# Fung-Lab/MatDeepLearn

Measured on AMD Instinct MI355X. Metric: edges/sec training CGCNN on bulk_data, higher is better.
Workload: dtype bf16

## Files before the change

include/mdl_hip.h:

```cpp
#ifndef MDL_HIP_H
#define MDL_HIP_H

#include <stddef.h>
#include <stdint.h>

#ifdef __cplusplus
extern "C" {
#endif

#define MDL_VERSION 100

enum { MDL_F32 = 0, MDL_BF16 = 1 };
enum { MDL_SUM = 0, MDL_MEAN = 1, MDL_MAX = 2 };
enum {
    MDL_OK = 0,
    MDL_E_ARG = -1,
    MDL_E_UNSUPP = -2,
    MDL_E_LAUNCH = -3
};

#define MDL_DTYPE_MASK 0xff
#define MDL_DETERMINISTIC 0x100
#define MDL_K3_PER_WAVE 0x200
#define MDL_K3_EDGE_LANE 0x400
#define MDL_BN_SHIFT_ROW 0x800
#define MDL_SPLIT_BF16 0x1000
#define MDL_MLP_F32_IO 0x2000

typedef void* mdlStream_t;

int mdl_version(void);
const char* mdl_last_error_string(void);
int mdl_debug_last_k3(void);

int mdl_rbf_expand(const float* d, const float* offsets, float coeff, void* out, int64_t E, int G,
                   int64_t ld_out, int out_dtype, mdlStream_t stream);

int mdl_csr_rowptr(const int32_t* sorted_index, int64_t E, int64_t N, int32_t* rowptr, mdlStream_t stream);

int mdl_segment_reduce_fwd(const void* src, const int32_t* rowptr, const int32_t* perm, void* out,
                           int32_t* argmax, int64_t N, int64_t C, int reduce, int dtype, mdlStream_t stream);
int mdl_segment_reduce_bwd(const void* grad_out, const int32_t* rowptr, const int32_t* seg,
                           const int32_t* perm, const int32_t* argmax, void* grad_src, int64_t N,
                           int64_t E, int64_t C, int reduce, int dtype, mdlStream_t stream);
int mdl_segment_reduce_bwd_add(const void* grad_out, const int32_t* rowptr, const int32_t* seg, const int32_t* perm,
                               const void* addend, void* grad_src, int64_t N, int64_t E, int64_t C, int reduce, int dtype,
                               mdlStream_t stream);

size_t mdl_cgconv_wpack_bytes(int C, int G, int dtype);
int mdl_cgconv_pack_weights(const float* w_f, const float* b_f, const float* w_s, const float* b_s, int C,
                            int G, void* wpack, float* bpack, int dtype, mdlStream_t stream);
int mdl_cgconv_pack_weights_node(const float* w_f, const float* b_f, const float* w_s, const float* b_s, int C,
                                 int G, void* wpack, float* bpack, void* wn_t, int dtype, mdlStream_t stream);

int mdl_cgconv_pack_weights_multi(int L, const float* const* w_f, const float* const* b_f, const float* const* w_s,
                                  const float* const* b_s, int C, int G, void* const* wpack, float* const* bpack,
                                  void* const* wn_t, int dtype, mdlStream_t stream);

int mdl_cgconv_fwd(const void* x, const void* edge_attr, const int32_t* rowptr, const int32_t* src,
                   const int32_t* tgt, const int32_t* eperm, const void* wpack, const float* bpack,
// ... 87 lines not shown
                       void* dh, void* dY, int64_t N, int Co, int D3, int dtype, mdlStream_t stream);

int mdl_pad_batch_tail(const int64_t* noff, const int64_t* eoff, int B, int64_t n_cap, int32_t* rowptr, int64_t* batch,
                       mdlStream_t stream);

int mdl_assemble_transposed(const int64_t* ids, const int64_t* noff, const int64_t* eoff, const int64_t* node_ptr,
                            const int64_t* edge_ptr, const int32_t* src_l, const int32_t* tgt_l, const int32_t* eperm_s,
                            const int32_t* lrowptr_s, int32_t* rowptr_s, int32_t* col_s, int32_t* eid_s, int32_t* src_s, int B,
                            int64_t n_cap, mdlStream_t stream);
int mdl_pad_edge_tail(const int64_t* noff, const int64_t* eoff, int B, int64_t n_cap, int64_t e_cap, int32_t* src, int32_t* tgt,
                      int32_t* col_s, int32_t* eid_s, int32_t* src_s, mdlStream_t stream);

int mdl_loss_fwd_bwd(const float* pred, const float* y, int64_t n, int kind, float* loss, float* grad, mdlStream_t stream);
int mdl_loss_fwd_bwd_rows(const float* pred, const float* y, int64_t n, int64_t n_total, int kind, float* loss, float* grad,
                          mdlStream_t stream);

#define MDL_BN_REPLICAS 16
int mdl_bn_sums_rows(void);
int mdl_bn_stats_n(const void* x, float* sums, int64_t N, int C, const int64_t* n_rows_dev, int dtype, mdlStream_t stream);
int mdl_bn_apply_n(const void* x, float* sums, const float* gamma, const float* beta, float* save, float* running_mean,
                   float* running_var, void* y, int64_t N, int C, float eps, float momentum, const int64_t* n_rows_dev,
                   int dtype, mdlStream_t stream);
int mdl_bn_bwd_stats_n(const void* dy, const void* x, const float* save, float* sums, int64_t N, int C,
                       const int64_t* n_rows_dev, int dtype, mdlStream_t stream);
int mdl_bn_bwd_apply_n(const void* dy, const void* x, const float* save, float* sums, const float* gamma, void* dx,
                       int64_t N, int C, const int64_t* n_rows_dev, int dtype, mdlStream_t stream);
int mdl_bn_bwd_apply_relu_n(const void* dy, const void* x, const float* save, float* sums, const float* gamma, void* dx,
                            int64_t N, int C, const int64_t* n_rows_dev, int dtype, mdlStream_t stream);
int mdl_linear_act(const void* x, const void* w, const void* bias, void* out, int64_t N, int K, int M, int act, int dtype,
                   mdlStream_t stream);
int mdl_linear_act_in(const void* x, const void* y, int xact, const void* w, const void* bias, void* out, int64_t N, int K,
                      int M, int act, int dtype, mdlStream_t stream);

int mdl_mlp_head_fwd(const void* x, const void* const* w, const void* const* b, void* const* h, int64_t N, int K0, int NL,
                     const int* M, int dtype, mdlStream_t stream);
int mdl_mlp_head_bwd(const void* x, const void* const* w, const void* const* h, const void* gy, void* dx, float* const* dw,
                     float* const* db, int64_t N, int K0, int NL, const int* M, int dtype, mdlStream_t stream);

int mdl_gru_gates_fwd(const void* gi, const void* gh, const float* h, float* h_out, void* out_lp, int64_t N, int C, int dtype,
                      mdlStream_t stream);
int mdl_gru_gates_bwd(const void* gi, const void* gh, const float* h, const float* g_h, const void* g_lp, void* dgi, void* dgh,
                      float* dh, int64_t N, int C, int dtype, mdlStream_t stream);

int mdl_linear_wide(const void* x, const void* w, void* out, int64_t N, int K, int64_t M, int dtype, mdlStream_t stream);

int mdl_gemm_tn(const void* a, int64_t lda, int M, const void* b, int64_t ldb, int K, float* c, int64_t N, int dtype,
                mdlStream_t stream);
int mdl_gemm_tn_colsum(const void* a, int64_t lda, int M, const void* b, int64_t ldb, int K, float* c, float* colsum,
                       int64_t N, int dtype, mdlStream_t stream);
int mdl_gemm_tn_act(const void* a, int64_t lda, int M, const void* y, int64_t ldy, int act, const void* b, int64_t ldb,
                    int K, float* c, float* colsum, int64_t N, int dtype, mdlStream_t stream);
int mdl_dense_bwd(const void* g, int64_t ldg, int M, const void* y, int64_t ldy, int act, const void* x, int64_t ldx, int K,
                  const void* w, void* dx, int64_t lddx, int xout, void* gm, float* dw, float* db, int64_t N, int dtype,
                  mdlStream_t stream);
size_t mdl_tn_scratch_bytes(void);
int mdl_dense_bwd_ex(const void* g, int64_t ldg, int M, const void* y, int64_t ldy, int act, const void* x, int64_t ldx, int K,
                     const void* w, void* dx, int64_t lddx, int xout, void* gm, float* dw, float* db, void* scratch, int64_t N,
                     int dtype, mdlStream_t stream);
int mdl_gemm_tn_ex(const void* a, int64_t lda, int M, const void* y, int64_t ldy, int act, const void* b, int64_t ldb, int K,
                   float* c, float* colsum, void* scratch, int64_t N, int dtype, mdlStream_t stream);

int mdl_gather_rows(const void* src, const int32_t* idx, void* out, int64_t E, int64_t C, int dtype,
                    mdlStream_t stream);
int mdl_gather_mul_reduce(const void* h, const void* w, const float* scale, const int32_t* rowptr,
                          const int32_t* col, const int32_t* eid, void* out, int64_t N, int64_t F, int reduce,
                          int dtype, mdlStream_t stream);
// ... 89 lines not shown
```

matdeeplearn_amd/_lib.py:

```python
import ctypes
import os

import torch

HERE = os.path.dirname(os.path.abspath(__file__))
LIB_PATH = os.path.join(HERE, "lib", "libmdl_hip.so")


def use_library(path):
    global LIB_PATH, _lib
    if _lib is not None and os.path.abspath(path) != os.path.abspath(LIB_PATH):
        raise MdlError("use_library(%s): %s is already loaded in this process" % (path, LIB_PATH))
    LIB_PATH = path

MDL_F32, MDL_BF16 = 0, 1
MDL_SUM, MDL_MEAN, MDL_MAX = 0, 1, 2
MDL_DTYPE_MASK, MDL_DETERMINISTIC, MDL_K3_PER_WAVE, MDL_K3_EDGE_LANE = 0xFF, 0x100, 0x200, 0x400
MDL_MLP_F32_IO = 0x2000
MDL_SPLIT_BF16 = 0x1000
MDL_BN_SHIFT_ROW = 0x800
MDL_BN_REPLICAS = 16
REDUCE = {"sum": MDL_SUM, "add": MDL_SUM, "mean": MDL_MEAN, "max": MDL_MAX}

_vp, _i64, _i32, _f32, _sz = ctypes.c_void_p, ctypes.c_int64, ctypes.c_int, ctypes.c_float, ctypes.c_size_t
_u32 = ctypes.c_uint32


class MdlCgConv(ctypes.Structure):
    _fields_ = [("size", _u32), ("dtype", _i32), ("flags", _u32), ("aggr", _i32), ("N", _i64), ("E", _i64), ("C", _i32), ("G", _i32),
                ("x", _vp), ("edge_attr", _vp), ("rowptr", _vp), ("src", _vp), ("tgt", _vp), ("eperm", _vp), ("wpack", _vp),
                ("bpack", _vp), ("out", _vp), ("bn_sums", _vp), ("bn_shift", _vp), ("bn_rows", _vp), ("grad_out", _vp),
                ("r_tgt", _vp), ("r_src", _vp), ("r_src_dtype", _i32), ("ld_dwe", _i32), ("dwe", _vp), ("db", _vp),
                ("workspace", _vp), ("workspace_bytes", _sz), ("balance", _vp)]


class MdlCgNode(ctypes.Structure):
    _fields_ = [("size", _u32), ("dtype", _i32), ("flags", _u32), ("zero_src", _i32), ("N", _i64), ("C", _i32), ("r_src_dtype", _i32),
                ("ld_dwn", _i32), ("reserved", _i32), ("x", _vp), ("grad_out", _vp), ("r_tgt", _vp), ("r_src", _vp), ("wn_t", _vp), ("dx", _vp), ("dwn", _vp)]


def _dp(t):
    return None if t is None else t.data_ptr()


def cg_args(**kw):
    a = MdlCgConv()
    a.size = ctypes.sizeof(MdlCgConv)
    for k, v in kw.items():
        setattr(a, k, _dp(v) if torch.is_tensor(v) else v)
    return a


def cg_node_args(**kw):
    a = MdlCgNode()
    a.size = ctypes.sizeof(MdlCgNode)
    for k, v in kw.items():
        setattr(a, k, _dp(v) if torch.is_tensor(v) else v)
    return a

PROTOTYPES = {
    "mdl_version": (_i32, []),
    "mdl_last_error_string": (ctypes.c_char_p, []),
    "mdl_debug_last_k3": (_i32, []),
    "mdl_rbf_expand": (_i32, [_vp, _vp, _f32, _vp, _i64, _i32, _i64, _i32, _vp]),
    "mdl_csr_rowptr": (_i32, [_vp, _i64, _i64, _vp, _vp]),
    "mdl_segment_reduce_fwd": (_i32, [_vp, _vp, _vp, _vp, _vp, _i64, _i64, _i32, _i32, _vp]),
    "mdl_segment_reduce_bwd": (_i32, [_vp, _vp, _vp, _vp, _vp, _vp, _i64, _i64, _i64, _i32, _i32, _vp]),
    "mdl_segment_reduce_bwd_add": (_i32, [_vp, _vp, _vp, _vp, _vp, _vp, _i64, _i64, _i64, _i32, _i32, _vp]),
    "mdl_cgconv_wpack_bytes": (_sz, [_i32, _i32, _i32]),
    "mdl_cgconv_pack_weights": (_i32, [_vp, _vp, _vp, _vp, _i32, _i32, _vp, _vp, _i32, _vp]),
    "mdl_cgconv_pack_weights_node": (_i32, [_vp, _vp, _vp, _vp, _i32, _i32, _vp, _vp, _vp, _i32, _vp]),
# ... 132 lines not shown
```

matdeeplearn_amd/csrc/mlp.hip:

```cpp
#include "mdl_common.h"

namespace mdl {

constexpr int MLP_MAXL = 4;
constexpr int MLP_LD = 72;

struct MlpArgs {
    const bf16_t* x;
    const bf16_t* w[MLP_MAXL];
    const bf16_t* b[MLP_MAXL];
    bf16_t* h[MLP_MAXL];
    const bf16_t* gy;
    bf16_t* dx;
    float* dw[MLP_MAXL];
    float* db[MLP_MAXL];
    int64_t N;
    int K0, NL;
    int M[MLP_MAXL];
    int f32io;
};

typedef __attribute__((ext_vector_type(4))) short s16x4;
typedef __attribute__((address_space(3))) s16x4* mlp_lds4_t;

__device__ __forceinline__ void mlp_stage(bf16_t* tile, const bf16_t* src, int64_t r0, int64_t N, int K, int tid) {
    if (K & 1) {
        bf16_t v[16];
#pragma unroll
        for (int u = 0; u < 16; ++u) {
            const int q = tid + 256 * u, row = q >> 6, c = q & 63;
            const bool ok = r0 + row < N && c < K;
            v[u] = src[ok ? (r0 + row) * (int64_t)K + c : 0];
        }
#pragma unroll
        for (int u = 0; u < 16; ++u) {
            const int q = tid + 256 * u, row = q >> 6, c = q & 63;
            tile[row * MLP_LD + c] = (r0 + row < N && c < K) ? v[u] : (bf16_t)0;
        }
        return;
    }
    const int k2 = K >> 1;
    unsigned v[8];
#pragma unroll
    for (int u = 0; u < 8; ++u) {
        const int q = tid + 256 * u, row = q >> 5, d = q & 31;
        const bool ok = r0 + row < N && d < k2;
        v[u] = *reinterpret_cast<const unsigned*>(src + (ok ? (r0 + row) * (int64_t)K + 2 * d : 0));
    }
#pragma unroll
    for (int u = 0; u < 8; ++u) {
        const int q = tid + 256 * u, row = q >> 5, d = q & 31;
        *reinterpret_cast<unsigned*>(tile + row * MLP_LD + 2 * d) = (r0 + row < N && d < k2) ? v[u] : 0u;
    }
}

__device__ __forceinline__ void mlp_stage_f32(bf16_t* tile, const float* src, int64_t r0, int64_t N, int K, int tid) {
    float v[16];
#pragma unroll
    for (int u = 0; u < 16; ++u) {
        const int q = tid + 256 * u, row = q >> 6, c = q & 63;
        const bool ok = r0 + row < N && c < K;
        v[u] = src[ok ? (r0 + row) * (int64_t)K + c : 0];
    }
#pragma unroll
    for (int u = 0; u < 16; ++u) {
        const int q = tid + 256 * u, row = q >> 6, c = q & 63;
        tile[row * MLP_LD + c] = (r0 + row < N && c < K) ? f2bf(v[u]) : (bf16_t)0;
    }
}

__device__ __forceinline__ f32x16 mlp_block(const bf16_t* tile_in, const bf16_t* wl, int mt, int nt, int i, int h, float bias) {
    f32x16 acc;
#pragma unroll
    for (int r = 0; r < 16; ++r) acc[r] = bias;
#pragma unroll
    for (int kk = 0; kk < 4; ++kk) {
        const bf16x8 a = *reinterpret_cast<const bf16x8*>(tile_in + (mt * 32 + i) * MLP_LD + 16 * kk + 8 * h);
        const bf16x8 b = *reinterpret_cast<const bf16x8*>(wl + (nt * 32 + i) * MLP_LD + 16 * kk + 8 * h);
        acc = __builtin_amdgcn_mfma_f32_32x32x16_bf16(a, b, acc, 0, 0, 0);
    }
    return acc;
}

__global__ __launch_bounds__(256, 2) void mlp_head_fwd_kernel(MlpArgs p) {
    extern __shared__ __attribute__((aligned(16))) char smem[];
    bf16_t* wl = reinterpret_cast<bf16_t*>(smem);
    bf16_t* ta = wl + p.NL * 64 * MLP_LD;
    bf16_t* tb = ta + 64 * MLP_LD;
    const int tid = threadIdx.x, lane = tid & 63, i = lane & 31, h = lane >> 5, wv = __builtin_amdgcn_readfirstlane(tid >> 6);
    const int mt = wv & 1, nt = wv >> 1;
    {
        unsigned wv_[MLP_MAXL][8];
#pragma unroll
        for (int l = 0; l < MLP_MAXL; ++l) {
            const int K = l < p.NL ? (l ? p.M[l - 1] : p.K0) : 0, M = l < p.NL ? p.M[l] : 0;
#pragma unroll
            for (int u = 0; u < 8; ++u) {
                const int q = tid + 256 * u, row = q >> 5, d = q & 31;
                unsigned v = 0u;
                if (row < M && 2 * d < K) v = *reinterpret_cast<const unsigned*>(p.w[l] + (int64_t)row * K + 2 * d);
                wv_[l][u] = v;
            }
        }
#pragma unroll
        for (int l = 0; l < MLP_MAXL; ++l) {
            if (l >= p.NL) break;
#pragma unroll
            for (int u = 0; u < 8; ++u) {
                const int q = tid + 256 * u, row = q >> 5, d = q & 31;
                *reinterpret_cast<unsigned*>(wl + (l * 64 + row) * MLP_LD + 2 * d) = wv_[l][u];
            }
        }
    }
    const int64_t n_tiles = (p.N + 63) / 64;
    for (int64_t tile = blockIdx.x; tile < n_tiles; tile += gridDim.x) {
        const int64_t r0 = tile * 64;
        __syncthreads();
        mlp_stage(ta, p.x, r0, p.N, p.K0, tid);
        __syncthreads();
        bf16_t* tin = ta;
        bf16_t* tout = tb;
        for (int l = 0; l < p.NL; ++l) {
            const int M = p.M[l], col = nt * 32 + i;
            const float bias = (p.b[l] && col < M) ? bf2f(p.b[l][col]) : 0.0f;
            const f32x16 acc = mlp_block(tin, wl + l * 64 * MLP_LD, mt, nt, i, h, bias);
            const bool relu = l + 1 < p.NL;
            bf16_t* const out = p.h[l];
            float* const out32 = (!relu && p.f32io) ? reinterpret_cast<float*>(p.h[l]) : nullptr;
#pragma unroll
            for (int r = 0; r < 16; ++r) {
                const int row = mt * 32 + 4 * h + (r & 3) + 8 * (r >> 2);
                float v = acc[r];
                if (relu) v = v > 0.0f ? v : 0.0f;
                const bf16_t hv = f2bf(v);
                tout[row * MLP_LD + col] = hv;
                if (col < M && r0 + row < p.N) {
                    if (out32) out32[(r0 + row) * (int64_t)M + col] = bf2f(hv);
                    else out[(r0 + row) * (int64_t)M + col] = hv;
                }
            }
            __syncthreads();
            bf16_t* t = tin; tin = tout; tout = t;
        }
    }
}

__global__ __launch_bounds__(256, 1) void mlp_head_bwd_kernel(MlpArgs p) {
    extern __shared__ __attribute__((aligned(16))) char smem[];
    bf16_t* wt = reinterpret_cast<bf16_t*>(smem);
    bf16_t* tin = wt + p.NL * 64 * MLP_LD;
    bf16_t* da = tin + p.NL * 64 * MLP_LD;
    bf16_t* dbuf = da + 64 * MLP_LD;
    const int tid = threadIdx.x, lane = tid & 63, i = lane & 31, h = lane >> 5, wv = __builtin_amdgcn_readfirstlane(tid >> 6);
    const int mt = wv & 1, nt = wv >> 1, t16 = i & 15;
    {
        unsigned wv_[MLP_MAXL][8];
#pragma unroll
        for (int l = 0; l < MLP_MAXL; ++l) {
            const int K = l < p.NL ? (l ? p.M[l - 1] : p.K0) : 0, M = l < p.NL ? p.M[l] : 0;
#pragma unroll
            for (int u = 0; u < 8; ++u) {
                const int q = tid + 256 * u, m = q >> 5, d = q & 31;
                unsigned v = 0u;
                if (m < M && 2 * d + 1 < K) v = *reinterpret_cast<const unsigned*>(p.w[l] + (int64_t)m * K + 2 * d);
                else if (m < M && 2 * d < K) v = (unsigned)p.w[l][(int64_t)m * K + 2 * d];
                wv_[l][u] = v;
            }
        }
#pragma unroll
        for (int l = 0; l < MLP_MAXL; ++l) {
            if (l >= p.NL) break;
#pragma unroll
            for (int u = 0; u < 8; ++u) {
                const int q = tid + 256 * u, m = q >> 5, d = q & 31;
                wt[(l * 64 + 2 * d) * MLP_LD + m] = (bf16_t)(wv_[l][u] & 0xffffu);
                wt[(l * 64 + 2 * d + 1) * MLP_LD + m] = (bf16_t)(wv_[l][u] >> 16);
            }
        }
    }
// ... 6 lines not shown
    const int64_t n_tiles = (p.N + 63) / 64;
    for (int64_t tile = blockIdx.x; tile < n_tiles; tile += gridDim.x) {
        const int64_t r0 = tile * 64;
        __syncthreads();
        for (int l = 0; l < p.NL; ++l)
            mlp_stage(tin + l * 64 * MLP_LD, l ? p.h[l - 1] : p.x, r0, p.N, l ? p.M[l - 1] : p.K0, tid);
        if (p.f32io) mlp_stage_f32(da, reinterpret_cast<const float*>(p.gy), r0, p.N, p.M[p.NL - 1], tid);
        else mlp_stage(da, p.gy, r0, p.N, p.M[p.NL - 1], tid);
        __syncthreads();
        bf16_t* dcur = da;
        bf16_t* dnext = dbuf;
#pragma unroll
        for (int lq = 0; lq < MLP_MAXL; ++lq) {
            const int l = p.NL - 1 - lq;
            if (l < 0) break;
            const bf16_t* const in = tin + l * 64 * MLP_LD;
#pragma unroll
            for (int ks = 0; ks < 4; ++ks) {
                const int roff = 16 * ks + 8 * h + (t16 >> 2), coff = (i & 16) + 4 * (t16 & 3);
                const bf16_t* pa = dcur + roff * MLP_LD + mt * 32 + coff;
                const bf16_t* pb = in + roff * MLP_LD + nt * 32 + coff;
                const s16x4 a0 = __builtin_amdgcn_ds_read_tr16_b64_v4i16((mlp_lds4_t)pa), a1 = __builtin_amdgcn_ds_read_tr16_b64_v4i16((mlp_lds4_t)(pa + 4 * MLP_LD));
                const s16x4 b0 = __builtin_amdgcn_ds_read_tr16_b64_v4i16((mlp_lds4_t)pb), b1 = __builtin_amdgcn_ds_read_tr16_b64_v4i16((mlp_lds4_t)(pb + 4 * MLP_LD));
                const bf16x8 af = {a0[0], a0[1], a0[2], a0[3], a1[0], a1[1], a1[2], a1[3]};
                const bf16x8 bf = {b0[0], b0[1], b0[2], b0[3], b1[0], b1[1], b1[2], b1[3]};
                dwacc[lq] = __builtin_amdgcn_mfma_f32_32x32x16_bf16(af, bf, dwacc[lq], 0, 0, 0);
            }
            {
                float s = 0.0f;
#pragma unroll
                for (int r = 0; r < 16; ++r) s += bf2f(dcur[(16 * (tid >> 6) + r) * MLP_LD + (tid & 63)]);
                dbacc[lq] += s;
            }
            if (l > 0 || p.dx) {
                const f32x16 acc = mlp_block(dcur, wt + l * 64 * MLP_LD, mt, nt, i, h, 0.0f);
                const int col = nt * 32 + i, K = l ? p.M[l - 1] : p.K0;
#pragma unroll
                for (int r = 0; r < 16; ++r) {
                    const int row = mt * 32 + 4 * h + (r & 3) + 8 * (r >> 2);
                    if (l > 0) {
                        const bool on = bf2f(in[row * MLP_LD + col]) > 0.0f;
                        dnext[row * MLP_LD + col] = f2bf(on ? acc[r] : 0.0f);
                    } else if (col < K && r0 + row < p.N) {
                        p.dx[(r0 + row) * (int64_t)K + col] = f2bf(acc[r]);
                    }
                }
            }
            __syncthreads();
            bf16_t* t = dcur; dcur = dnext; dnext = t;
        }
    }
    {
        float* red = reinterpret_cast<float*>(da);
        __syncthreads();
#pragma unroll
        for (int lq = 0; lq < MLP_MAXL; ++lq) red[(lq * 4 + (tid >> 6)) * 64 + (tid & 63)] = dbacc[lq];
        __syncthreads();
#pragma unroll
        for (int lq = 0; lq < MLP_MAXL; ++lq)
            dbacc[lq] = tid < 64 ? ((red[(lq * 4 + 0) * 64 + tid] + red[(lq * 4 + 1) * 64 + tid]) + red[(lq * 4 + 2) * 64 + tid]) + red[(lq * 4 + 3) * 64 + tid] : 0.0f;
    }
#pragma unroll
    for (int lq = 0; lq < MLP_MAXL; ++lq) {
        const int l = p.NL - 1 - lq;
        if (l < 0) break;
        const int K = l ? p.M[l - 1] : p.K0, M = p.M[l], k = nt * 32 + i;
#pragma unroll
        for (int r = 0; r < 16; ++r) {
            const int m = mt * 32 + 4 * h + (r & 3) + 8 * (r >> 2);
            if (m < M && k < K) unsafeAtomicAdd(p.dw[l] + (int64_t)m * K + k, dwacc[lq][r]);
        }
        if (tid < 64 && tid < M && p.db[l]) unsafeAtomicAdd(p.db[l] + tid, dbacc[lq]);
    }
}

static int mlp_check(const char* name, const MlpArgs& a, int dtype) {
    MDL_REQUIRE(dtype == MDL_BF16, MDL_E_UNSUPP, "%s: bf16 only", name);
    MDL_REQUIRE(a.NL >= 1 && a.NL <= MLP_MAXL && a.K0 >= 2 && a.K0 <= 64 && a.K0 % 2 == 0, MDL_E_UNSUPP,
                "%s: 1..4 dense layers, even input width <= 64 (got %d layers, K0 = %d)", name, a.NL, a.K0);
    for (int l = 0; l < a.NL; ++l) {
        MDL_REQUIRE(a.M[l] >= 1 && a.M[l] <= 64 && (l + 1 == a.NL || a.M[l] % 2 == 0), MDL_E_UNSUPP,
                    "%s: widths <= 64, hidden widths even (layer %d: %d)", name, l, a.M[l]);
        MDL_REQUIRE(a.w[l] && reinterpret_cast<uintptr_t>(a.w[l]) % 4 == 0, MDL_E_ARG, "%s: null / misaligned weight %d", name, l);
    }
    MDL_REQUIRE(a.N >= 0 && (a.N == 0 || (a.x && reinterpret_cast<uintptr_t>(a.x) % 4 == 0)), MDL_E_ARG, "%s: bad arguments", name);
    return MDL_OK;
}

}

extern "C" int mdl_mlp_head_fwd(const void* x, const void* const* w, const void* const* b, void* const* h, int64_t N, int K0,
                                int NL, const int* M, int dtype, mdlStream_t stream) {
    using namespace mdl;
    MlpArgs a = {};
    a.x = (const bf16_t*)x; a.N = N; a.K0 = K0; a.NL = NL;
    MDL_REQUIRE(NL >= 1 && NL <= MLP_MAXL && w && b && h && M, MDL_E_ARG, "mdl_mlp_head_fwd: bad arguments");
    for (int l = 0; l < NL; ++l) { a.w[l] = (const bf16_t*)w[l]; a.b[l] = (const bf16_t*)b[l]; a.h[l] = (bf16_t*)h[l]; a.M[l] = M[l]; }
    a.f32io = (dtype & MDL_MLP_F32_IO) != 0;
    dtype &= MDL_DTYPE_MASK;
    int rc = mlp_check("mdl_mlp_head_fwd", a, dtype);
    if (rc) return rc;
    for (int l = 0; l < NL; ++l) MDL_REQUIRE(N == 0 || a.h[l], MDL_E_ARG, "mdl_mlp_head_fwd: null output %d", l);
    if (N == 0) return MDL_OK;
    const int lds = (NL + 2) * 64 * MLP_LD * 2;
    hipError_t e = set_max_dynamic_lds(reinterpret_cast<const void*>(mlp_head_fwd_kernel), lds);
    if (e != hipSuccess) { set_error("mdl_mlp_head_fwd: LDS attribute (%d B): %s", lds, hipGetErrorString(e)); return MDL_E_LAUNCH; }
    int64_t grid = cdiv(N, 64);
    if (grid > 512) grid = 512;
    hipLaunchKernelGGL(mlp_head_fwd_kernel, dim3((unsigned)grid), dim3(256), lds, (hipStream_t)stream, a);
    return check_launch("mdl_mlp_head_fwd");
}

extern "C" int mdl_mlp_head_bwd(const void* x, const void* const* w, const void* const* h, const void* gy, void* dx,
                                float* const* dw, float* const* db, int64_t N, int K0, int NL, const int* M, int dtype,
                                mdlStream_t stream) {
    using namespace mdl;
    MlpArgs a = {};
    a.x = (const bf16_t*)x; a.gy = (const bf16_t*)gy; a.dx = (bf16_t*)dx; a.N = N; a.K0 = K0; a.NL = NL;
    MDL_REQUIRE(NL >= 1 && NL <= MLP_MAXL && w && h && dw && db && M, MDL_E_ARG, "mdl_mlp_head_bwd: bad arguments");
    for (int l = 0; l < NL; ++l) {
        a.w[l] = (const bf16_t*)w[l]; a.M[l] = M[l]; a.dw[l] = dw[l]; a.db[l] = db[l];
        a.h[l] = l + 1 < NL ? (bf16_t*)const_cast<void*>(h[l]) : nullptr;
    }
    const bool det = (dtype & MDL_DETERMINISTIC) != 0;
    a.f32io = (dtype & MDL_MLP_F32_IO) != 0;
    dtype &= MDL_DTYPE_MASK;
    int rc = mlp_check("mdl_mlp_head_bwd", a, dtype);
    if (rc) return rc;
    MDL_REQUIRE(N == 0 || (gy && reinterpret_cast<uintptr_t>(gy) % ((M[NL - 1] % 2 && !a.f32io) ? 2 : 4) == 0), MDL_E_ARG,
                "mdl_mlp_head_bwd: null / misaligned gy");
    for (int l = 0; l < NL; ++l) {
        MDL_REQUIRE(N == 0 || a.dw[l], MDL_E_ARG, "mdl_mlp_head_bwd: null dw %d", l);
        MDL_REQUIRE(N == 0 || l + 1 == NL || (a.h[l] && reinterpret_cast<uintptr_t>(a.h[l]) % 4 == 0), MDL_E_ARG, "mdl_mlp_head_bwd: null h %d", l);
    }
    if (N == 0) return MDL_OK;
    const int lds = (2 * NL + 2) * 64 * MLP_LD * 2;
    hipError_t e = set_max_dynamic_lds(reinterpret_cast<const void*>(mlp_head_bwd_kernel), lds);
    if (e != hipSuccess) { set_error("mdl_mlp_head_bwd: LDS attribute (%d B): %s", lds, hipGetErrorString(e)); return MDL_E_LAUNCH; }
    int64_t grid = cdiv(N, 64);
    if (grid > 256) grid = 256;
    if (det) grid = 1;
    hipLaunchKernelGGL(mlp_head_bwd_kernel, dim3((unsigned)grid), dim3(256), lds, (hipStream_t)stream, a);
    return check_launch("mdl_mlp_head_bwd");
}
```

matdeeplearn_amd/models/_base.py:

```python
import torch
import torch.nn.functional as F
from torch import nn

from .. import ops
from ..nn import BatchNorm1d, Set2Set, lowp_copies as _lowp


def dense(lin, h, split=False):
    if h.dtype == lin.weight.dtype:
        if split and ops.linear_split_ok(h, lin.weight):
            return ops._LinearSplitTN.apply(h, lin.weight, lin.bias)
        return lin(h)
    return ops.linear(h, lin.weight, lin.bias, _lowp(lin))


def dense_act(lin, h, act, split=False):
    if h.dtype == lin.weight.dtype:
        return getattr(F, act)(dense(lin, h, split))
    return ops.linear_act(h, lin.weight, lin.bias, act, _lowp(lin))


class GraphModel(nn.Module):

    def _begin(self, data, dim1, pre_fc_count, gc_count, pool, pool_order, batch_norm, batch_track_stats, act,
# ... 75 lines not shown
        ops.new_grad_arena(device, n)

    def _pre(self, out):
        if torch.is_grad_enabled() and out.is_cuda:
            self._open_grad_arena(out.device)
        if out.dtype == torch.bfloat16 and torch.is_grad_enabled():
            self._cast_dense(out.dtype)
        for lin in self.pre_lin_list:
            out = dense_act(lin, out, self.act, split=self.split_products)
        return out

    def _bn(self, i, out):
        return self.bn_list[i](out) if self.batch_norm == "True" else out

    def _drop(self, out):
        return F.dropout(out, p=self.dropout_rate, training=self.training)

    def _post(self, out, final=False):
        lins = list(self.post_lin_list) + [self.lin_out]
        if out.dtype != self.lin_out.weight.dtype and ops.mlp_head_ok(out, lins, self.act):
            return ops.mlp_head(out, lins, [_lowp(lin) for lin in lins], f32_out=final)
        for lin in self.post_lin_list:
            out = dense_act(lin, out, self.act, split=self.split_products)
        return dense(self.lin_out, out)

    def _pool(self, out, data):
        num_graphs = getattr(data, "num_graphs", None)
        if self.pool == "set2set":
            return self.set2set(out, data.batch, num_graphs)
        return ops.POOLS[self.pool](out, data.batch, num_graphs, seg_index=getattr(data, "pool_index", None))

    def _head(self, out, data):
        if self.pool_order == "early":
            out = self._post(self._pool(out, data).to(out.dtype), final=True)
        else:
            out = self._post(out)
            if self.pool == "set2set":
                out = dense(self.lin_out_2, self._pool(out, data).to(out.dtype))
            else:
                out = self._pool(out, data)
        out = out.float()
        return out.view(-1) if out.shape[1] == 1 else out
```

matdeeplearn_amd/ops.py:

```python
import collections
import os
import weakref

import torch

from . import _lib
from ._lib import MdlError, check, dtype_code, lib, ptr, require_hip, stream

_ACT_CODE = {"relu": 1, "ssp": 2}
_LN2 = 0.6931471805599453


def _f32c(t):
    return None if t is None else t.detach().float().contiguous()


def _stream_key(device):
    return (device.index, torch.cuda.current_stream(device).cuda_stream)


class EdgeCSR:

    __slots__ = ("rowptr", "src", "tgt", "eperm", "N", "E", "_row", "_col", "_t", "_attr", "_tb", "_bal", "partial", "__weakref__")

# ... 484 lines not shown
    prev, _DET = _DET, bool(on)
    return prev


class deterministic:
    def __init__(self, on=True):
        self.on = on

    def __enter__(self):
        self.prev = set_deterministic(self.on)
        return self

    def __exit__(self, *exc):
        set_deterministic(self.prev)
        return False


OPTIONS = {
    "deterministic": ("_DET", "bit-reproducible launch shapes of every atomically accumulating kernel (slow; HIP-vs-HIP tests)"),
    "gmr_dw": ("_GMR_DW", "CFConv backward: dh and dw from one walk over the by-source CSR"),
    "balance": ("_BALANCE", "cost-balanced node ranges for the edge-per-lane CGConv backward (E >= 4e5)"),
    "pad128": ("_PAD128", "C in (96, 128): static 128-channel CGConv kernels on zero-padded rows"),
    "rsrc16": ("_RSRC16", "by-source sums of the CGConv backward in bf16 (packed atomics)"),
    "cg_bn_stats": ("_CG_BN_STATS", "BatchNorm statistics in the CGConv forward's epilogue (measured time-neutral: off)"),
    "direct_grads": ("_DIRECT_GRADS", "K3 / K3c add into the final dW layout (measured slower at small batches: off)"),
    "cfconv_fused": ("_CFCONV_FUSED", "K4: the fused CFConv forward"),
    "cfconv_recompute": ("_CFCONV_RECOMPUTE", "K4b: CFConv backward with the filter recomputed (no per-edge activations)"),
    "tn_colsum": ("_TN_COLSUM", "bias gradients out of the TN GEMM"),
    "dense_bwd": ("_DENSE_BWD", "dX + dW + db of a tall dense layer in one pass"),
    "dense_bwd_wide": ("_DENSE_BWD_WIDE", "... also when both widths exceed 128"),
    "mlp_head": ("_MLP_HEAD", "post-FC head as one launch per direction"),
    "linear_wide": ("_LINEAR_WIDE", "NNConv's Y = x W2r on the streaming kernel"),
    "set2set_fused": ("_SET2SET_FUSED", "Set2Set readout: all processing steps in one launch per direction (off: torch's LSTM + the composed attention)"),
    "tn_scratch": ("_TN_SCRATCH", "weight-gradient blocks of the TN products as plain stores + a reduce launch (off: atomics from every workgroup)"),
}


def configure(**kw):
    prev = {}
    g = globals()
    for k, v in kw.items():
        if k not in OPTIONS:
            raise MdlError("ops.configure: unknown option %r (known: %s)" % (k, ", ".join(sorted(OPTIONS))))
        attr = OPTIONS[k][0]
        prev[k] = g[attr]
        g[attr] = bool(v)
    return prev


def options():
    return {k: globals()[a] for k, (a, _) in OPTIONS.items()}


def _dflag():
    return _lib.MDL_DETERMINISTIC if _DET else 0


K3_VARIANT = None


def _k3flag():
    return {None: 0, "per_wave": _lib.MDL_K3_PER_WAVE, "edge_lane": _lib.MDL_K3_EDGE_LANE}[K3_VARIANT]


def last_k3():
    return int(lib().mdl_debug_last_k3())
# ... 1008 lines not shown
            flat, dbv = _dw_db_zeros(M[l], Ks[l], x.device)
            dws.append(flat.view(M[l], Ks[l]))
            dbs.append(dbv if ctx.has_bias[l] else None)
        dx = torch.empty_like(x) if ctx.needs_input_grad[0] else None
        Ma = (ctypes.c_int * NL)(*M)
        check(lib().mdl_mlp_head_bwd(ptr(x), _ptr_array(ws), _ptr_array(hs + [None]), ptr(gy), ptr(dx), _ptr_array(dws), _ptr_array(dbs),
                                     N, K0, NL, Ma, dtype_code(x) | _dflag() | ctx.io, stream()), "mdl_mlp_head_bwd")
        grads = []
        for l in range(NL):
            grads.append(dws[l].to(ctx.wdtypes[l]))
            grads.append(dbs[l].to(ctx.wdtypes[l]) if ctx.has_bias[l] else None)
        return (dx, None, None) + tuple(grads)


def mlp_head_ok(x, lins, act):
    if not (_MLP_HEAD and act == "relu" and x.dtype == torch.bfloat16 and x.is_cuda and x.dim() == 2 and x.is_contiguous()
            and 1 <= len(lins) <= 4 and x.shape[0] >= 1 and x.shape[1] <= 64 and x.shape[1] % 2 == 0 and x.data_ptr() % 4 == 0):
        return False
    k = x.shape[1]
    for j, lin in enumerate(lins):
        if lin.in_features != k or lin.out_features > 64 or (j + 1 < len(lins) and lin.out_features % 2) or not lin.weight.requires_grad:
            return False
        k = lin.out_features
    return True


def mlp_head(x, lins, lowp=None, f32_out=False):
    params = []
    for lin in lins:
        params += [lin.weight, lin.bias]
    return _MlpHead.apply(x, lowp, bool(f32_out), *params)


class _LinearWide(torch.autograd.Function):

    @staticmethod
    def forward(ctx, x, w):
        N, K = x.shape
        M = w.shape[1]
        wt = w.t().contiguous()
        out = torch.empty((N, M), dtype=x.dtype, device=x.device)
        check(lib().mdl_linear_wide(ptr(x), ptr(wt), ptr(out), N, K, M, dtype_code(x), stream()), "mdl_linear_wide")
        ctx.save_for_backward(x, w)
        return out

    @staticmethod
    def backward(ctx, g):
        x, w = ctx.saved_tensors
        dx = g @ w.t() if ctx.needs_input_grad[0] else None
        dw = x.t() @ g if ctx.needs_input_grad[1] else None
        return dx, dw


def matmul_wide(x, w):
    if (_LINEAR_WIDE and x.dtype == torch.bfloat16 and w.dtype == torch.bfloat16 and x.is_cuda and x.dim() == 2 and x.is_contiguous()
            and x.shape[0] >= 1024 and x.shape[1] % 2 == 0 and 4 <= x.shape[1] <= 160 and w.shape[1] >= 640
            and x.data_ptr() % 16 == 0):
        return _LinearWide.apply(x, w)
    return x @ w


def linear_act_fused_ok(x, weight, act):
    return (x.dtype == torch.bfloat16 and x.is_cuda and x.dim() == 2 and x.is_contiguous() and x.shape[0] >= _DENSE_MIN_ROWS
            and _fused_fwd_shape_ok(weight.shape[0], weight.shape[1], act) and x.data_ptr() % 16 == 0 and weight.requires_grad)


# ... 872 lines not shown
```

Measured before the change: 819.8 million.

## Fuse graph pooling into the MLP head kernels for forward and backward

Adds an MDL_MLP_POOL mode in which the MLP head forward kernel sums or averages each graph's node rows straight into its LDS tile, using 512 threads where the extra waves help with the gather. The backward kernel scatters the first-layer input gradient back to the node rows. This removes the separate segment-reduce launch and its backward, along with the pooled-tensor round trips. The cost is a larger forward block with half the waves idle during the GEMM stage, and an imbalanced per-graph node loop.

Result: no change. 822.7 million, median of 6 (+0.4%).

```diff
diff --git a/include/mdl_hip.h b/include/mdl_hip.h
--- a/include/mdl_hip.h
+++ b/include/mdl_hip.h
@@ -26,6 +26,7 @@
 #define MDL_BN_SHIFT_ROW 0x800
 #define MDL_SPLIT_BF16 0x1000
 #define MDL_MLP_F32_IO 0x2000
+#define MDL_MLP_POOL 0x4000
 
 typedef void* mdlStream_t;
 
@@ -179,6 +180,14 @@
 int mdl_linear_act_in(const void* x, const void* y, int xact, const void* w, const void* bias, void* out, int64_t N, int K,
                       int M, int act, int dtype, mdlStream_t stream);
 
+typedef struct MdlReadout {
+    uint32_t size;
+    int32_t pool;
+    int64_t n_nodes;
+    const int32_t* node_ptr;
+    const void* x;
+    void* pooled;
+} MdlReadout;
 int mdl_mlp_head_fwd(const void* x, const void* const* w, const void* const* b, void* const* h, int64_t N, int K0, int NL,
                      const int* M, int dtype, mdlStream_t stream);
 int mdl_mlp_head_bwd(const void* x, const void* const* w, const void* const* h, const void* gy, void* dx, float* const* dw,
diff --git a/matdeeplearn_amd/_lib.py b/matdeeplearn_amd/_lib.py
--- a/matdeeplearn_amd/_lib.py
+++ b/matdeeplearn_amd/_lib.py
@@ -17,6 +17,7 @@
 MDL_SUM, MDL_MEAN, MDL_MAX = 0, 1, 2
 MDL_DTYPE_MASK, MDL_DETERMINISTIC, MDL_K3_PER_WAVE, MDL_K3_EDGE_LANE = 0xFF, 0x100, 0x200, 0x400
 MDL_MLP_F32_IO = 0x2000
+MDL_MLP_POOL = 0x4000
 MDL_SPLIT_BF16 = 0x1000
 MDL_BN_SHIFT_ROW = 0x800
 MDL_BN_REPLICAS = 16
@@ -37,6 +38,17 @@
 class MdlCgNode(ctypes.Structure):
     _fields_ = [("size", _u32), ("dtype", _i32), ("flags", _u32), ("zero_src", _i32), ("N", _i64), ("C", _i32), ("r_src_dtype", _i32),
                 ("ld_dwn", _i32), ("reserved", _i32), ("x", _vp), ("grad_out", _vp), ("r_tgt", _vp), ("r_src", _vp), ("wn_t", _vp), ("dx", _vp), ("dwn", _vp)]
+
+
+class MdlReadout(ctypes.Structure):
+    _fields_ = [("size", _u32), ("pool", _i32), ("n_nodes", _i64), ("node_ptr", _vp), ("x", _vp), ("pooled", _vp)]
+
+
+def readout_args(pool, n_nodes, node_ptr, x, pooled):
+    a = MdlReadout()
+    a.size, a.pool, a.n_nodes = ctypes.sizeof(MdlReadout), pool, n_nodes
+    a.node_ptr, a.x, a.pooled = _dp(node_ptr), _dp(x), _dp(pooled)
+    return a
 
 
 def _dp(t):
diff --git a/matdeeplearn_amd/csrc/mlp.hip b/matdeeplearn_amd/csrc/mlp.hip
--- a/matdeeplearn_amd/csrc/mlp.hip
+++ b/matdeeplearn_amd/csrc/mlp.hip
@@ -18,7 +18,15 @@
     int K0, NL;
     int M[MLP_MAXL];
     int f32io;
+    const int32_t* node_ptr;
+    const bf16_t* xn;
+    bf16_t* pooled;
+    bf16_t* dxn;
+    int64_t NN;
+    int mean;
 };
+
+typedef __attribute__((ext_vector_type(4))) unsigned mlp_u32x4;
 
 typedef __attribute__((ext_vector_type(4))) short s16x4;
 typedef __attribute__((address_space(3))) s16x4* mlp_lds4_t;
@@ -54,6 +62,76 @@
     }
 }
 
+template <int NT>
+__device__ __forceinline__ void mlp_stage_pool(bf16_t* tile, const MlpArgs& p, int64_t r0, int tid) {
+    constexpr int S = 512 / NT, U = 16 / S;
+    int b[S], n[S];
+    float acc[S][8];
+#pragma unroll
+    for (int s = 0; s < S; ++s) {
+        const int g = (tid + NT * s) >> 3;
+        const bool ok = r0 + g < p.N;
+        const int64_t lo = ok ? p.node_ptr[r0 + g] : 0, hi = ok ? p.node_ptr[r0 + g + 1] : 0;
+        b[s] = (int)(lo < 0 ? 0 : (lo > p.NN ? p.NN : lo));
+        n[s] = (int)((hi > p.NN ? p.NN : hi) - b[s]);
+        if (n[s] < 0) n[s] = 0;
+#pragma unroll
+        for (int j = 0; j < 8; ++j) acc[s][j] = 0.0f;
+    }
+    const bf16_t* const base = p.xn + (tid & 7) * 8;
+    const int nmax = n[0] > n[S - 1] ? n[0] : n[S - 1];
+    for (int k = 0; k < nmax; k += U) {
+        bf16x8 v[S][U];
+#pragma unroll
+        for (int s = 0; s < S; ++s)
+#pragma unroll
+            for (int u = 0; u < U; ++u) {
+                int kk = b[s] + (k + u < n[s] ? k + u : n[s] - 1);
+                if (kk < 0) kk = 0;
+                v[s][u] = *reinterpret_cast<const bf16x8*>(base + (int64_t)kk * 64);
+            }
+#pragma unroll
+        for (int s = 0; s < S; ++s)
+#pragma unroll
+            for (int u = 0; u < U; ++u)
+                if (k + u < n[s]) {
+#pragma unroll
+                    for (int j = 0; j < 8; ++j) acc[s][j] += bf2f((bf16_t)v[s][u][j]);
+                }
+    }
+#pragma unroll
+    for (int s = 0; s < S; ++s) {
+        const int q = tid + NT * s, g = q >> 3, c8 = q & 7;
+        if (p.mean) {
+            const float cnt = (float)(n[s] > 1 ? n[s] : 1);
+#pragma unroll
+            for (int j = 0; j < 8; ++j) acc[s][j] = acc[s][j] / cnt;
+        }
+        const mlp_u32x4 r = {pk_bf16(acc[s][0], acc[s][1]), pk_bf16(acc[s][2], acc[s][3]), pk_bf16(acc[s][4], acc[s][5]), pk_bf16(acc[s][6], acc[s][7])};
+        *reinterpret_cast<mlp_u32x4*>(tile + g * MLP_LD + c8 * 8) = r;
+        if (r0 + g < p.N) *reinterpret_cast<mlp_u32x4*>(p.pooled + (r0 + g) * 64 + c8 * 8) = r;
+    }
+}
+
+__device__ __forceinline__ void mlp_unpool(const bf16_t* tile, const MlpArgs& p, int64_t r0, int tid) {
+#pragma unroll
+    for (int s = 0; s < 2; ++s) {
+        const int q = tid + 256 * s, g = q >> 3, c8 = q & 7;
+        if (r0 + g >= p.N) continue;
+        const int64_t lo = p.node_ptr[r0 + g], hi = p.node_ptr[r0 + g + 1];
+        const int64_t b = lo < 0 ? 0 : (lo > p.NN ? p.NN : lo), e = hi > p.NN ? p.NN : hi;
+        float v[8];
+        Vec<bf16_t>::ld(tile + g * MLP_LD + c8 * 8, v);
+        if (p.mean) {
+            const float cnt = (float)(e - b > 1 ? e - b : 1);
+#pragma unroll
+            for (int j = 0; j < 8; ++j) v[j] = v[j] / cnt;
+        }
+        const mlp_u32x4 r = {pk_bf16(v[0], v[1]), pk_bf16(v[2], v[3]), pk_bf16(v[4], v[5]), pk_bf16(v[6], v[7])};
+        for (int64_t k = b; k < e; ++k) *reinterpret_cast<mlp_u32x4*>(p.dxn + k * 64 + c8 * 8) = r;
+    }
+}
+
 __device__ __forceinline__ void mlp_stage_f32(bf16_t* tile, const float* src, int64_t r0, int64_t N, int K, int tid) {
     float v[16];
 #pragma unroll
@@ -82,14 +160,15 @@
     return acc;
 }
 
-__global__ __launch_bounds__(256, 2) void mlp_head_fwd_kernel(MlpArgs p) {
+template <bool POOL>
+__global__ __launch_bounds__(POOL ? 512 : 256, POOL ? 1 : 2) void mlp_head_fwd_kernel(MlpArgs p) {
     extern __shared__ __attribute__((aligned(16))) char smem[];
     bf16_t* wl = reinterpret_cast<bf16_t*>(smem);
     bf16_t* ta = wl + p.NL * 64 * MLP_LD;
     bf16_t* tb = ta + 64 * MLP_LD;
     const int tid = threadIdx.x, lane = tid & 63, i = lane & 31, h = lane >> 5, wv = __builtin_amdgcn_readfirstlane(tid >> 6);
     const int mt = wv & 1, nt = wv >> 1;
-    {
+    if (!POOL || tid < 256) {
         unsigned wv_[MLP_MAXL][8];
 #pragma unroll
         for (int l = 0; l < MLP_MAXL; ++l) {
@@ -116,27 +195,30 @@
     for (int64_t tile = blockIdx.x; tile < n_tiles; tile += gridDim.x) {
         const int64_t r0 = tile * 64;
         __syncthreads();
-        mlp_stage(ta, p.x, r0, p.N, p.K0, tid);
+        if constexpr (POOL) mlp_stage_pool<512>(ta, p, r0, tid);
+        else mlp_stage(ta, p.x, r0, p.N, p.K0, tid);
         __syncthreads();
         bf16_t* tin = ta;
         bf16_t* tout = tb;
         for (int l = 0; l < p.NL; ++l) {
             const int M = p.M[l], col = nt * 32 + i;
-            const float bias = (p.b[l] && col < M) ? bf2f(p.b[l][col]) : 0.0f;
-            const f32x16 acc = mlp_block(tin, wl + l * 64 * MLP_LD, mt, nt, i, h, bias);
             const bool relu = l + 1 < p.NL;
             bf16_t* const out = p.h[l];
             float* const out32 = (!relu && p.f32io) ? reinterpret_cast<float*>(p.h[l]) : nullptr;
-#pragma unroll
-            for (int r = 0; r < 16; ++r) {
-                const int row = mt * 32 + 4 * h + (r & 3) + 8 * (r >> 2);
-                float v = acc[r];
-                if (relu) v = v > 0.0f ? v : 0.0f;
-                const bf16_t hv = f2bf(v);
-                tout[row * MLP_LD + col] = hv;
-                if (col < M && r0 + row < p.N) {
-                    if (out32) out32[(r0 + row) * (int64_t)M + col] = bf2f(hv);
-                    else out[(r0 + row) * (int64_t)M + col] = hv;
+            if (!POOL || wv < 4) {
+                const float bias = (p.b[l] && col < M) ? bf2f(p.b[l][col]) : 0.0f;
+                const f32x16 acc = mlp_block(tin, wl + l * 64 * MLP_LD, mt, nt, i, h, bias);
+#pragma unroll
+                for (int r = 0; r < 16; ++r) {
+                    const int row = mt * 32 + 4 * h + (r & 3) + 8 * (r >> 2);
+                    float v = acc[r];
+                    if (relu) v = v > 0.0f ? v : 0.0f;
+                    const bf16_t hv = f2bf(v);
+                    tout[row * MLP_LD + col] = hv;
+                    if (col < M && r0 + row < p.N) {
+                        if (out32) out32[(r0 + row) * (int64_t)M + col] = bf2f(hv);
+                        else out[(r0 + row) * (int64_t)M + col] = hv;
+                    }
                 }
             }
             __syncthreads();
@@ -145,6 +227,7 @@
     }
 }
 
+template <bool POOL>
 __global__ __launch_bounds__(256, 1) void mlp_head_bwd_kernel(MlpArgs p) {
     extern __shared__ __attribute__((aligned(16))) char smem[];
     bf16_t* wt = reinterpret_cast<bf16_t*>(smem);
@@ -217,7 +300,7 @@
                 for (int r = 0; r < 16; ++r) s += bf2f(dcur[(16 * (tid >> 6) + r) * MLP_LD + (tid & 63)]);
                 dbacc[lq] += s;
             }
-            if (l > 0 || p.dx) {
+            if (l > 0 || p.dx || POOL) {
                 const f32x16 acc = mlp_block(dcur, wt + l * 64 * MLP_LD, mt, nt, i, h, 0.0f);
                 const int col = nt * 32 + i, K = l ? p.M[l - 1] : p.K0;
 #pragma unroll
@@ -226,6 +309,8 @@
                     if (l > 0) {
                         const bool on = bf2f(in[row * MLP_LD + col]) > 0.0f;
                         dnext[row * MLP_LD + col] = f2bf(on ? acc[r] : 0.0f);
+                    } else if constexpr (POOL) {
+                        dnext[row * MLP_LD + col] = f2bf(acc[r]);
                     } else if (col < K && r0 + row < p.N) {
                         p.dx[(r0 + row) * (int64_t)K + col] = f2bf(acc[r]);
                     }
@@ -234,6 +319,7 @@
             __syncthreads();
             bf16_t* t = dcur; dcur = dnext; dnext = t;
         }
+        if constexpr (POOL) mlp_unpool(dcur, p, r0, tid);
     }
     {
         float* red = reinterpret_cast<float*>(da);
@@ -274,57 +360,100 @@
 
 }
 
-extern "C" int mdl_mlp_head_fwd(const void* x, const void* const* w, const void* const* b, void* const* h, int64_t N, int K0,
-                                int NL, const int* M, int dtype, mdlStream_t stream) {
+static int mlp_fwd_launch(const char* name, mdl::MlpArgs& a, const void* const* w, const void* const* b, void* const* h, int NL,
+                          const int* M, int dtype, bool pool, mdlStream_t stream) {
     using namespace mdl;
-    MlpArgs a = {};
-    a.x = (const bf16_t*)x; a.N = N; a.K0 = K0; a.NL = NL;
-    MDL_REQUIRE(NL >= 1 && NL <= MLP_MAXL && w && b && h && M, MDL_E_ARG, "mdl_mlp_head_fwd: bad arguments");
+    MDL_REQUIRE(NL >= 1 && NL <= MLP_MAXL && w && b && h && M, MDL_E_ARG, "%s: bad arguments", name);
+    a.NL = NL;
     for (int l = 0; l < NL; ++l) { a.w[l] = (const bf16_t*)w[l]; a.b[l] = (const bf16_t*)b[l]; a.h[l] = (bf16_t*)h[l]; a.M[l] = M[l]; }
     a.f32io = (dtype & MDL_MLP_F32_IO) != 0;
     dtype &= MDL_DTYPE_MASK;
-    int rc = mlp_check("mdl_mlp_head_fwd", a, dtype);
+    int rc = mlp_check(name, a, dtype);
     if (rc) return rc;
-    for (int l = 0; l < NL; ++l) MDL_REQUIRE(N == 0 || a.h[l], MDL_E_ARG, "mdl_mlp_head_fwd: null output %d", l);
+    for (int l = 0; l < NL; ++l) MDL_REQUIRE(a.N == 0 || a.h[l], MDL_E_ARG, "%s: null output %d", name, l);
+    if (a.N == 0) return MDL_OK;
+    const int lds = (NL + 2) * 64 * MLP_LD * 2;
+    auto kf = pool ? mlp_head_fwd_kernel<true> : mlp_head_fwd_kernel<false>;
+    hipError_t e = set_max_dynamic_lds(reinterpret_cast<const void*>(kf), lds);
+    if (e != hipSuccess) { set_error("%s: LDS attribute (%d B): %s", name, lds, hipGetErrorString(e)); return MDL_E_LAUNCH; }
+    int64_t grid = cdiv(a.N, 64);
+    if (grid > 512) grid = 512;
+    hipLaunchKernelGGL(kf, dim3((unsigned)grid), dim3(pool ? 512 : 256), lds, (hipStream_t)stream, a);
+    return check_launch(name);
+}
+
+static int readout_args(const char* name, const MdlReadout* r, const void* rows, int64_t B, int K0, mdl::MlpArgs& a) {
+    using namespace mdl;
+    MDL_REQUIRE(r && r->size == sizeof(MdlReadout), MDL_E_ARG, "%s: MDL_MLP_POOL needs x = an MdlReadout of this layout (size %u, expected %u)",
+                name, r ? r->size : 0u, (unsigned)sizeof(MdlReadout));
+    MDL_REQUIRE(r->pool == MDL_SUM || r->pool == MDL_MEAN, MDL_E_UNSUPP, "%s: MdlReadout.pool must be MDL_SUM or MDL_MEAN (got %d)", name, r->pool);
+    MDL_REQUIRE(K0 == 64, MDL_E_UNSUPP, "%s: MDL_MLP_POOL needs K0 = 64 (got %d)", name, K0);
+    MDL_REQUIRE(B >= 0 && r->n_nodes >= 1 && r->n_nodes < (1ll << 31) && rows && r->node_ptr && (B == 0 || r->pooled), MDL_E_ARG,
+                "%s: MDL_MLP_POOL: bad arguments", name);
+    MDL_REQUIRE(reinterpret_cast<uintptr_t>(rows) % 16 == 0 && reinterpret_cast<uintptr_t>(r->pooled) % 16 == 0, MDL_E_ARG,
+                "%s: MDL_MLP_POOL: node rows and pooled rows must be 16-byte aligned", name);
+    a.x = (const bf16_t*)r->pooled; a.N = B; a.K0 = 64;
+    a.node_ptr = r->node_ptr; a.NN = r->n_nodes; a.mean = r->pool == MDL_MEAN;
+    return MDL_OK;
+}
+
+extern "C" int mdl_mlp_head_fwd(const void* x, const void* const* w, const void* const* b, void* const* h, int64_t N, int K0,
+                                int NL, const int* M, int dtype, mdlStream_t stream) {
+    mdl::MlpArgs a = {};
+    if (dtype & MDL_MLP_POOL) {
+        const MdlReadout* r = static_cast<const MdlReadout*>(x);
+        int rc = readout_args("mdl_mlp_head_fwd", r, r ? r->x : nullptr, N, K0, a);
+        if (rc) return rc;
+        a.xn = (const mdl::bf16_t*)r->x; a.pooled = (mdl::bf16_t*)r->pooled;
+        return mlp_fwd_launch("mdl_mlp_head_fwd", a, w, b, h, NL, M, dtype & ~MDL_MLP_POOL, true, stream);
+    }
+    a.x = (const mdl::bf16_t*)x; a.N = N; a.K0 = K0;
+    return mlp_fwd_launch("mdl_mlp_head_fwd", a, w, b, h, NL, M, dtype, false, stream);
+}
+
+static int mlp_bwd_launch(const char* name, mdl::MlpArgs& a, const void* const* w, const void* const* h, const void* gy,
+                          float* const* dw, float* const* db, int NL, const int* M, int dtype, bool pool, mdlStream_t stream) {
+    using namespace mdl;
+    const int64_t N = a.N;
+    a.gy = (const bf16_t*)gy; a.NL = NL;
+    MDL_REQUIRE(NL >= 1 && NL <= MLP_MAXL && w && h && dw && db && M, MDL_E_ARG, "%s: bad arguments", name);
+    for (int l = 0; l < NL; ++l) {
+        a.w[l] = (const bf16_t*)w[l]; a.M[l] = M[l]; a.dw[l] = dw[l]; a.db[l] = db[l];
+        a.h[l] = l + 1 < NL ? (bf16_t*)const_cast<void*>(h[l]) : nullptr;
+    }
+    const bool det = (dtype & MDL_DETERMINISTIC) != 0;
+    a.f32io = (dtype & MDL_MLP_F32_IO) != 0;
+    dtype &= MDL_DTYPE_MASK;
+    int rc = mlp_check(name, a, dtype);
+    if (rc) return rc;
+    MDL_REQUIRE(N == 0 || (gy && reinterpret_cast<uintptr_t>(gy) % ((M[NL - 1] % 2 && !a.f32io) ? 2 : 4) == 0), MDL_E_ARG,
+                "%s: null / misaligned gy", name);
+    for (int l = 0; l < NL; ++l) {
+        MDL_REQUIRE(N == 0 || a.dw[l], MDL_E_ARG, "%s: null dw %d", name, l);
+        MDL_REQUIRE(N == 0 || l + 1 == NL || (a.h[l] && reinterpret_cast<uintptr_t>(a.h[l]) % 4 == 0), MDL_E_ARG, "%s: null h %d", name, l);
+    }
     if (N == 0) return MDL_OK;
-    const int lds = (NL + 2) * 64 * MLP_LD * 2;
-    hipError_t e = set_max_dynamic_lds(reinterpret_cast<const void*>(mlp_head_fwd_kernel), lds);
-    if (e != hipSuccess) { set_error("mdl_mlp_head_fwd: LDS attribute (%d B): %s", lds, hipGetErrorString(e)); return MDL_E_LAUNCH; }
+    const int lds = (2 * NL + 2) * 64 * MLP_LD * 2;
+    auto kf = pool ? mlp_head_bwd_kernel<true> : mlp_head_bwd_kernel<false>;
+    hipError_t e = set_max_dynamic_lds(reinterpret_cast<const void*>(kf), lds);
+    if (e != hipSuccess) { set_error("%s: LDS attribute (%d B): %s", name, lds, hipGetErrorString(e)); return MDL_E_LAUNCH; }
     int64_t grid = cdiv(N, 64);
-    if (grid > 512) grid = 512;
-    hipLaunchKernelGGL(mlp_head_fwd_kernel, dim3((unsigned)grid), dim3(256), lds, (hipStream_t)stream, a);
-    return check_launch("mdl_mlp_head_fwd");
+    if (grid > 256) grid = 256;
+    if (det) grid = 1;
+    hipLaunchKernelGGL(kf, dim3((unsigned)grid), dim3(256), lds, (hipStream_t)stream, a);
+    return check_launch(name);
 }
 
 extern "C" int mdl_mlp_head_bwd(const void* x, const void* const* w, const void* const* h, const void* gy, void* dx,
                                 float* const* dw, float* const* db, int64_t N, int K0, int NL, const int* M, int dtype,
                                 mdlStream_t stream) {
-    using namespace mdl;
-    MlpArgs a = {};
-    a.x = (const bf16_t*)x; a.gy = (const bf16_t*)gy; a.dx = (bf16_t*)dx; a.N = N; a.K0 = K0; a.NL = NL;
-    MDL_REQUIRE(NL >= 1 && NL <= MLP_MAXL && w && h && dw && db && M, MDL_E_ARG, "mdl_mlp_head_bwd: bad arguments");
-    for (int l = 0; l < NL; ++l) {
-        a.w[l] = (const bf16_t*)w[l]; a.M[l] = M[l]; a.dw[l] = dw[l]; a.db[l] = db[l];
-        a.h[l] = l + 1 < NL ? (bf16_t*)const_cast<void*>(h[l]) : nullptr;
-    }
-    const bool det = (dtype & MDL_DETERMINISTIC) != 0;
-    a.f32io = (dtype & MDL_MLP_F32_IO) != 0;
-    dtype &= MDL_DTYPE_MASK;
-    int rc = mlp_check("mdl_mlp_head_bwd", a, dtype);
-    if (rc) return rc;
-    MDL_REQUIRE(N == 0 || (gy && reinterpret_cast<uintptr_t>(gy) % ((M[NL - 1] % 2 && !a.f32io) ? 2 : 4) == 0), MDL_E_ARG,
-                "mdl_mlp_head_bwd: null / misaligned gy");
-    for (int l = 0; l < NL; ++l) {
-        MDL_REQUIRE(N == 0 || a.dw[l], MDL_E_ARG, "mdl_mlp_head_bwd: null dw %d", l);
-        MDL_REQUIRE(N == 0 || l + 1 == NL || (a.h[l] && reinterpret_cast<uintptr_t>(a.h[l]) % 4 == 0), MDL_E_ARG, "mdl_mlp_head_bwd: null h %d", l);
-    }
-    if (N == 0) return MDL_OK;
-    const int lds = (2 * NL + 2) * 64 * MLP_LD * 2;
-    hipError_t e = set_max_dynamic_lds(reinterpret_cast<const void*>(mlp_head_bwd_kernel), lds);
-    if (e != hipSuccess) { set_error("mdl_mlp_head_bwd: LDS attribute (%d B): %s", lds, hipGetErrorString(e)); return MDL_E_LAUNCH; }
-    int64_t grid = cdiv(N, 64);
-    if (grid > 256) grid = 256;
-    if (det) grid = 1;
-    hipLaunchKernelGGL(mlp_head_bwd_kernel, dim3((unsigned)grid), dim3(256), lds, (hipStream_t)stream, a);
-    return check_launch("mdl_mlp_head_bwd");
-}
+    mdl::MlpArgs a = {};
+    if (dtype & MDL_MLP_POOL) {
+        int rc = readout_args("mdl_mlp_head_bwd", static_cast<const MdlReadout*>(x), dx, N, K0, a);
+        if (rc) return rc;
+        a.dxn = (mdl::bf16_t*)dx;
+        return mlp_bwd_launch("mdl_mlp_head_bwd", a, w, h, gy, dw, db, NL, M, dtype & ~MDL_MLP_POOL, true, stream);
+    }
+    a.x = (const mdl::bf16_t*)x; a.dx = (mdl::bf16_t*)dx; a.N = N; a.K0 = K0;
+    return mlp_bwd_launch("mdl_mlp_head_bwd", a, w, h, gy, dw, db, NL, M, dtype, false, stream);
+}
diff --git a/matdeeplearn_amd/models/_base.py b/matdeeplearn_amd/models/_base.py
--- a/matdeeplearn_amd/models/_base.py
+++ b/matdeeplearn_amd/models/_base.py
@@ -131,7 +131,15 @@
 
     def _head(self, out, data):
         if self.pool_order == "early":
-            out = self._post(self._pool(out, data).to(out.dtype), final=True)
+            lins = list(self.post_lin_list) + [self.lin_out]
+            si = None
+            if out.dtype != self.lin_out.weight.dtype and self.pool in ops.POOLS:
+                si = ops.readout_ok(out, data.batch, getattr(data, "num_graphs", None), getattr(data, "pool_index", None), self.pool,
+                                    lins, self.act)
+            if si is not None:
+                out = ops.readout(out, si, self.pool, lins, [_lowp(lin) for lin in lins], f32_out=True)
+            else:
+                out = self._post(self._pool(out, data).to(out.dtype), final=True)
         else:
             out = self._post(out)
             if self.pool == "set2set":
diff --git a/matdeeplearn_amd/ops.py b/matdeeplearn_amd/ops.py
--- a/matdeeplearn_amd/ops.py
+++ b/matdeeplearn_amd/ops.py
@@ -540,6 +540,8 @@
     "mlp_head": ("_MLP_HEAD", "post-FC head as one launch per direction"),
     "linear_wide": ("_LINEAR_WIDE", "NNConv's Y = x W2r on the streaming kernel"),
     "set2set_fused": ("_SET2SET_FUSED", "Set2Set readout: all processing steps in one launch per direction (off: torch's LSTM + the composed attention)"),
+    "readout": ("_READOUT", "pool + post-FC head as one launch per direction (off: segment reduce and head separately)"),
+    "readout_fwd": ("_READOUT_FWD", "... the forward launch of it (off: segment reduce + head forward, fused backward)"),
     "tn_scratch": ("_TN_SCRATCH", "weight-gradient blocks of the TN products as plain stores + a reduce launch (off: atomics from every workgroup)"),
 }
 
@@ -1614,6 +1616,89 @@
     return _MlpHead.apply(x, lowp, bool(f32_out), *params)
 
 
+_READOUT = True
+_READOUT_FWD = True
+
+
+class _Readout(torch.autograd.Function):
+
+    @staticmethod
+    def forward(ctx, x, si, reduce, lowp, f32_out, *params):
+        import ctypes
+        NL = len(params) // 2
+        wb = [_wb(x, params[2 * l], params[2 * l + 1], *((None, None) if lowp is None or lowp[l] is None else lowp[l]))
+              for l in range(NL)]
+        ws, bs = [w.contiguous() for w, _ in wb], [b for _, b in wb]
+        B, N = si.N, x.shape[0]
+        M = [int(w.shape[0]) for w in ws]
+        pooled = torch.empty((B, 64), dtype=x.dtype, device=x.device)
+        hs = [torch.empty((B, m), dtype=torch.float32 if (f32_out and l == NL - 1) else x.dtype, device=x.device)
+              for l, m in enumerate(M)]
+        Ma = (ctypes.c_int * NL)(*M)
+        io = _lib.MDL_MLP_F32_IO if f32_out else 0
+        if _READOUT_FWD:
+            rd = _lib.readout_args(reduce, N, si.rowptr, x, pooled)
+            check(lib().mdl_mlp_head_fwd(ctypes.cast(ctypes.pointer(rd), ctypes.c_void_p), _ptr_array(ws), _ptr_array(bs), _ptr_array(hs), B, 64, NL, Ma,
+                                         dtype_code(x) | io | _lib.MDL_MLP_POOL, stream()), "mdl_mlp_head_fwd (MDL_MLP_POOL)")
+        else:
+            check(lib().mdl_segment_reduce_fwd(ptr(x), ptr(si.rowptr), None, ptr(pooled), None, B, 64, reduce, dtype_code(x), stream()),
+                  "mdl_segment_reduce_fwd")
+            check(lib().mdl_mlp_head_fwd(ptr(pooled), _ptr_array(ws), _ptr_array(bs), _ptr_array(hs), B, 64, NL, Ma, dtype_code(x) | io,
+                                         stream()), "mdl_mlp_head_fwd")
+        ctx.save_for_backward(pooled, *ws, *hs[:-1])
+        ctx.si, ctx.reduce, ctx.NL, ctx.M, ctx.io, ctx.N = si, reduce, NL, M, io, N
+        ctx.has_bias = [params[2 * l + 1] is not None for l in range(NL)]
+        ctx.wdtypes = [params[2 * l].dtype for l in range(NL)]
+        return hs[-1]
+
+    @staticmethod
+    def backward(ctx, gy):
+        import ctypes
+        saved = ctx.saved_tensors
+        NL, M, si = ctx.NL, ctx.M, ctx.si
+        pooled, ws, hs = saved[0], list(saved[1:1 + NL]), list(saved[1 + NL:])
+        gy = gy.contiguous()
+        if gy.dtype != (torch.float32 if ctx.io else pooled.dtype):
+            gy = gy.to(torch.float32 if ctx.io else pooled.dtype)
+        Ks = [64] + M[:-1]
+        dws, dbs = [], []
+        for l in range(NL):
+            flat, dbv = _dw_db_zeros(M[l], Ks[l], pooled.device)
+            dws.append(flat.view(M[l], Ks[l]))
+            dbs.append(dbv if ctx.has_bias[l] else None)
+        dx = torch.empty((ctx.N, 64), dtype=pooled.dtype, device=pooled.device)
+        Ma = (ctypes.c_int * NL)(*M)
+        rd = _lib.readout_args(ctx.reduce, ctx.N, si.rowptr, None, pooled)
+        check(lib().mdl_mlp_head_bwd(ctypes.cast(ctypes.pointer(rd), ctypes.c_void_p), _ptr_array(ws), _ptr_array(hs + [None]), ptr(gy), ptr(dx),
+                                     _ptr_array(dws), _ptr_array(dbs), si.N, 64, NL, Ma, dtype_code(pooled) | ctx.io | _lib.MDL_MLP_POOL, stream()),
+              "mdl_mlp_head_bwd (MDL_MLP_POOL)")
+        grads = []
+        for l in range(NL):
+            grads.append(dws[l].to(ctx.wdtypes[l]))
+            grads.append(dbs[l].to(ctx.wdtypes[l]) if ctx.has_bias[l] else None)
+        return (dx, None, None, None, None) + tuple(grads)
+
+
+def readout_ok(x, batch, num_graphs, seg_index, pool, lins, act):
+    if not (_READOUT and not _DET and pool in ("global_mean_pool", "global_add_pool") and x.dim() == 2 and x.shape[1] == 64
+            and x.shape[0] >= 1 and x.is_cuda and x.dtype == torch.bfloat16 and x.data_ptr() % 16 == 0 and mlp_head_ok(x, lins, act)):
+        return None
+    if seg_index is None:
+        if num_graphs is None:
+            return None
+        seg_index = _seg_index(batch, num_graphs, True)
+    if seg_index.partial or seg_index.perm is not None or seg_index.E != x.shape[0] or seg_index.N < 1:
+        return None
+    return seg_index
+
+
+def readout(x, seg_index, pool, lins, lowp=None, f32_out=False):
+    params = []
+    for lin in lins:
+        params += [lin.weight, lin.bias]
+    return _Readout.apply(x, seg_index, _lib.MDL_MEAN if pool == "global_mean_pool" else _lib.MDL_SUM, lowp, bool(f32_out), *params)
+
+
 class _LinearWide(torch.autograd.Function):
 
     @staticmethod
```
